# iclavera/learning_to_adapt

Hardware: AMD Instinct MI355X
Metric: controller-steps/sec (n_cand=2000, H=30, ens=5) (higher is better)
Workload: dtype f32

## Files before the change

learning_to_adapt_amd/csrc/l2a_mfma.h:

```cpp
#pragma once

#include <type_traits>

#include "l2a_kernels.h"

#ifndef L2A_XEARLY
#define L2A_XEARLY 1
#endif

#ifndef L2A_NW
#define L2A_NW 4
#endif

typedef unsigned int u32x4 __attribute__((ext_vector_type(4)));
__device__ __forceinline__ __amdgpu_buffer_rsrc_t l2a_rsrc(const void* base, long long bytes) {
    return __builtin_amdgcn_make_buffer_rsrc(const_cast<void*>(base), 0, (int)bytes, 0x00020000);
}
__device__ __forceinline__ f32x4 l2a_ldw(__amdgpu_buffer_rsrc_t rs, int voff, int soff) {
    return __builtin_bit_cast(f32x4, __builtin_amdgcn_raw_buffer_load_b128(rs, voff, soff, 0));
}

template <bool GACT>
__device__ __forceinline__ f32x4 l2a_actv(f32x4 v, int kind, float floor) {
    if (GACT) return l2a_act4(v, kind);
    v.x = l2a_max_nan(v.x, floor); v.y = l2a_max_nan(v.y, floor);
    v.z = l2a_max_nan(v.z, floor); v.w = l2a_max_nan(v.w, floor);
    return v;
}

__device__ __forceinline__ float l2a_sum_xor16(float x) {
    const unsigned int u = __float_as_uint(x);
    const auto r = __builtin_amdgcn_permlane16_swap(u, u, false, false);
    return __uint_as_float(r[0]) + __uint_as_float(r[1]);
}
__device__ __forceinline__ float l2a_sum_xor32(float x) {
    const unsigned int u = __float_as_uint(x);
    const auto r = __builtin_amdgcn_permlane32_swap(u, u, false, false);
    return __uint_as_float(r[0]) + __uint_as_float(r[1]);
}

#define L2A_MFMA4(a, b, c) __builtin_amdgcn_mfma_f32_4x4x1f32((a), (b), (c), 0, 0, 0)

#define L2A_OPAQUE(v) asm volatile("" : "+v"(v))

#ifndef L2A_TIMELINE
#define L2A_TS(slot)
#else
#define L2A_TS(slot)                                                                        \
    if (p.dbg && pairid == 0 && e < 8 && grp < 2) {                                         \
        unsigned long long ts_;                                                             \
        asm volatile("s_memtime %0\n\ts_waitcnt lgkmcnt(0)" : "=s"(ts_) : : "memory");       \
        if (lane == 0) p.dbg[(((long long)(grp * p.h + t) * 8 + e) * 8 + wave) * 16 + (slot)] = ts_; \
    }
#endif

#define L2A_STAGE_MFMA(CA, CB)                                                             \
    _Pragma("unroll") for (int ii = 0; ii < 4; ++ii)                                       \
        _Pragma("unroll") for (int nt = 0; nt < NT; ++nt)                                  \
            _Pragma("unroll") for (int tt = TW - 1; tt >= 0; --tt)    \
                acc[nt][tt] = L2A_MFMA(CA[tt][ii], CB[nt][ii], acc[nt][tt]);

#define L2A_STAGE(CA, CB, FA, FB, SOFF, IMM, GF)                                           \
    {                                                                                      \
        _Pragma("unroll") for (int tt = 0; tt < TW; ++tt)                                  \
            FA[tt] = l2a_ldw(rs, voff[tt] + (IMM), (SOFF));                                \
        _Pragma("unroll") for (int nt = 0; nt < NT; ++nt)                                  \
            FB[nt] = hin[(nt * HT + (GF)) * 64 + lane];                                    \
        L2A_STAGE_MFMA(CA, CB)                                                             \
         \
        __builtin_amdgcn_sched_group_barrier(0x100, NT, 0);                                \
        _Pragma("unroll") for (int tt = 0; tt < TW; ++tt) {                                \
            __builtin_amdgcn_sched_group_barrier(0x008, 4 * NT, 0);                        \
            __builtin_amdgcn_sched_group_barrier(0x020, 1, 0);                             \
        }                                                                                  \
        __builtin_amdgcn_sched_barrier(0);                                                 \
    }

#define L2A_PFT_MAX 6
#define L2A_PFT(TW_, OT_) ((OT_) <= 2 ? ((TW_) < L2A_PFT_MAX ? (TW_) : L2A_PFT_MAX) : ((TW_) < 2 ? (TW_) : 2))

template <int NT, int TW, int TPW, int OT, bool LAST>
__device__ __forceinline__ void l2a_hidden_gemm(__amdgpu_buffer_rsrc_t rs, __amdgpu_buffer_rsrc_t rsn,
                                                const int (&voff)[TPW], const int (&voffn)[TPW], int twn,
                                                int tile0, const f32x4* hin,
                                                f32x4 (&aA)[TPW], f32x4 (&aB)[TPW],
                                                f32x4 (&pfO)[TPW][OT], f32x4 (&acc)[NT][TPW], int lane,
                                                const float* bias_lds, f32x4 (&bias)[TPW], const int (&olane)[OT]) {
    constexpr int HT = L2A_NW * TPW;
    static_assert(HT % 4 == 0, "the k-group pipeline is unrolled by 4");
    f32x4 aC[TW], aD[TW], bA[NT], bB[NT], bC[NT], bD[NT];
#pragma unroll
    for (int nt = 0; nt < NT; ++nt) {
        bA[nt] = hin[(nt * HT + 0) * 64 + lane];
        bB[nt] = hin[(nt * HT + 1) * 64 + lane];
#pragma unroll
        for (int tt = 0; tt < TW; ++tt) acc[nt][tt] = (f32x4){0.f, 0.f, 0.f, 0.f};
    }
#pragma unroll
    for (int nt = 0; nt < NT; ++nt) { L2A_OPAQUE(bA[nt]); L2A_OPAQUE(bB[nt]); }
    __builtin_amdgcn_sched_barrier(0);

#pragma unroll 1
    for (int g = 0; g < HT - 4; g += 4) {
        const int soff = (g + 2) * 1024;
        L2A_STAGE(aA, bA, aC, bC, soff, 0, g + 2)
        L2A_STAGE(aB, bB, aD, bD, soff, 1024, g + 3)
        L2A_STAGE(aC, bC, aA, bA, soff, 2048, g + 4)
        L2A_STAGE(aD, bD, aB, bB, soff, 3072, g + 5)
    }
    L2A_STAGE(aA, bA, aC, bC, (HT - 2) * 1024, 0, HT - 2)
    L2A_STAGE(aB, bB, aD, bD, (HT - 2) * 1024, 1024, HT - 1)
    {
        if (LAST) {
#pragma unroll
            for (int tt = 0; tt < L2A_PFT(TW, OT); ++tt)
#pragma unroll
                for (int c = 0; c < OT; ++c)
                    if (((tt * OT + c) & 1) == 0)
                        pfO[tt][c] = l2a_ldw(rsn, olane[c] + (tile0 + tt) * 1024, c * HT * 1024);
        } else {
#pragma unroll
            for (int tt = 0; tt < TPW; ++tt)
                if (tt < twn) aA[tt] = l2a_ldw(rsn, voffn[tt], 0);
        }
        L2A_STAGE_MFMA(aC, bC)
        __builtin_amdgcn_sched_barrier(0);
    }
    {
#pragma unroll
        for (int tt = 0; tt < TW; ++tt) bias[tt] = *reinterpret_cast<const f32x4*>(bias_lds + 16 * tt);
        if (LAST) {
#pragma unroll
            for (int tt = 0; tt < L2A_PFT(TW, OT); ++tt)
#pragma unroll
                for (int c = 0; c < OT; ++c)
                    if (((tt * OT + c) & 1) == 1)
                        pfO[tt][c] = l2a_ldw(rsn, olane[c] + (tile0 + tt) * 1024, c * HT * 1024);
        } else {
#pragma unroll
            for (int tt = 0; tt < TPW; ++tt)
                if (tt < twn) aB[tt] = l2a_ldw(rsn, voffn[tt] + 1024, 0);
        }
        L2A_STAGE_MFMA(aD, bD)
        __builtin_amdgcn_sched_barrier(0);
    }
}

template <int NT, int TW, int TPW, int OT, int NPF, bool O4, class PF>
__device__ __forceinline__ void l2a_out_phase(const f32x4 (&hreg)[NT][TPW], f32x4 (&pfO)[TPW][OT],
                                              __amdgpu_buffer_rsrc_t rs_out, int tile0, PF prefetch,
                                              f32x4* pbuf, int chunk0, int lane, const int (&olane)[OT]) {
    constexpr int HT = L2A_NW * TPW;
    constexpr int CS = TPW / 2;
    constexpr int NCH = TW / CS;
    f32x4 a[TW][OT];
#pragma unroll
    for (int tt = 0; tt < TW; ++tt)
#pragma unroll
        for (int c = 0; c < OT; ++c)
            a[tt][c] = (tt < L2A_PFT(TW, OT)) ? pfO[tt][c]
                                              : l2a_ldw(rs_out, olane[c] + (tile0 + tt) * 1024, c * HT * 1024);
    prefetch();
    f32x4 acc[NCH][NT][OT];
#pragma unroll
    for (int ch = 0; ch < NCH; ++ch)
#pragma unroll
        for (int nt = 0; nt < NT; ++nt)
#pragma unroll
            for (int c = 0; c < OT; ++c) acc[ch][nt][c] = (f32x4){0.f, 0.f, 0.f, 0.f};
#pragma unroll
    for (int t2 = 0; t2 < CS; ++t2)
#pragma unroll
        for (int ii = 0; ii < 4; ++ii)
#pragma unroll
            for (int ch = 0; ch < NCH; ++ch)
#pragma unroll
                for (int nt = 0; nt < NT; ++nt)
#pragma unroll
                    for (int c = 0; c < OT; ++c)
                        acc[ch][nt][c] = (O4 && c == OT - 1)
                            ? L2A_MFMA4(a[ch * CS + t2][c][ii], hreg[nt][ch * CS + t2][ii], acc[ch][nt][c])
                            : L2A_MFMA(a[ch * CS + t2][c][ii], hreg[nt][ch * CS + t2][ii], acc[ch][nt][c]);
    {
        constexpr int NLATE = (TW - L2A_PFT(TW, OT)) * OT;
        constexpr int NMFMA = TW * 4 * NT * OT;
#pragma unroll
        for (int i = 0; i < NLATE; ++i) {
            __builtin_amdgcn_sched_group_barrier(0x020, 1, 0);
            __builtin_amdgcn_sched_group_barrier(0x008, 2, 0);
        }
        constexpr int PER = (NMFMA - 2 * NLATE) / NPF > 0 ? (NMFMA - 2 * NLATE) / NPF : 1;
#pragma unroll
        for (int i = 0; i < NPF; ++i) {
            __builtin_amdgcn_sched_group_barrier(0x008, PER, 0);
            __builtin_amdgcn_sched_group_barrier(0x020, 1, 0);
        }
    }
#pragma unroll
    for (int nt = 0; nt < NT; ++nt)
#pragma unroll
        for (int c = 0; c < OT; ++c)
            pbuf[((chunk0 * NT + nt) * OT + c) * 64 + lane] = (NCH == 2) ? acc[0][nt][c] + acc[NCH - 1][nt][c] : acc[0][nt][c];
}

template <int NT, int TPW, int OT, int KG0, bool GACT, int K0L = 4, bool N1 = false, bool O4 = false, bool FAN = false, bool WHOLE = false>
__global__ void __launch_bounds__(64 * L2A_NW) l2a_rollout_mfma_k(const L2AKParams p) {
    static_assert(!(FAN && WHOLE), "an instance is general, member fan or whole-tiles-only");
    constexpr bool NOHALF = FAN || WHOLE;
    constexpr int HT = L2A_NW * TPW;
    constexpr int TH = TPW / 2;
    static_assert(TPW % 2 == 0, "half members split a wave's tiles in two");
    constexpr int CST_BOUT = 32 * KG0 + 32 * OT;
    constexpr int CST_BHID = CST_BOUT + 16 * OT;
    constexpr int PS = L2A_NW * NT * OT * 64;
    const int NRM_SET = p.cst_set;
    const int LB = p.lb;
    extern __shared__ __attribute__((aligned(16))) char l2a_smem[];
    f32x4* buf0 = reinterpret_cast<f32x4*>(l2a_smem);
    f32x4* buf1 = buf0 + p.sa_elems;
    f32x4* pbase = buf0 + (LB > 1 ? LB : 2) * p.sa_elems;
    float* nrm = reinterpret_cast<float*>(buf0 + p.cst_off);

    const int tid = threadIdx.x;
    const int lane = tid & 63;
    const int wave = __builtin_amdgcn_readfirstlane(tid >> 6);
    const int jc = lane & 15;
    const int qq = lane >> 4;
    const int c0 = wave * TPW;
    int olane[OT];
#pragma unroll
    for (int c = 0; c < OT; ++c) olane[c] = ((O4 && c == OT - 1) ? ((lane & 48) | (lane & 3)) : lane) * 16;

    const int tail = p.split_from >= 0;
    const int in_tail = tail && (int)blockIdx.x >= p.split_from;
    const int split = FAN ? 3 : WHOLE ? 0 : (tail ? (in_tail ? p.split : 0) : p.split);
    const int n_tiles = p.m * p.tiles_per_env;
    const int n_pairs = tail ? n_tiles - p.split_from : n_tiles;
    int bid, grp, lpair, pairid;
    if (!tail && p.pl_units > 0) {
        const int hx = (int)blockIdx.x & 7, idx = (int)blockIdx.x >> 3;
        const int xcd = hx;
        const int f = p.pl_f, wide = p.pl_r * (f + 1);
        int u, k, xu;
        if (xcd < wide) { u = xcd / (f + 1); k = xcd - u * (f + 1); xu = f + 1; }
        else { const int y = xcd - wide; u = y / f; k = y - u * f; u += p.pl_r; xu = f; }
        const int su = (p.pl_w + xu - 1) / xu;
        const int j = k * su + idx;
        if (idx >= su || j >= p.pl_w) return;
        if (p.mode == L2A_MODE_PER_BLOCK) {
            grp = split ? j / p.tiles_per_env : 0;
            lpair = u * p.tiles_per_env + (j - grp * p.tiles_per_env);
        } else {
            grp = u;
            lpair = j;
        }
        bid = grp * n_pairs + lpair;
        pairid = lpair;
    } else if (!tail) {
        bid = l2a_logical_wg(blockIdx.x, gridDim.x);
        grp = split ? (bid / n_pairs) : 0;
        lpair = bid - grp * n_pairs;
        pairid = lpair;
    } else if (!in_tail) {
        bid = l2a_logical_wg(blockIdx.x, p.split_from);
        grp = 0; lpair = 0; pairid = bid;
    } else {
        bid = (int)blockIdx.x - p.split_from;
        grp = bid & 1; lpair = bid >> 1;
        pairid = p.split_from + lpair;
    }
#if defined(L2A_TIMELINE) || defined(L2A_WGREC)
    unsigned long long wg_t0_, wg_r0_;
    asm volatile("s_memtime %0\n\ts_memrealtime %1\n\ts_waitcnt lgkmcnt(0)" : "=s"(wg_t0_), "=s"(wg_r0_) : : "memory");
#endif
    const int env = pairid / p.tiles_per_env;
    const int tb = pairid - env * p.tiles_per_env;
    const int R = p.m * p.n;
    const int obs_dim = p.obs_dim, act_dim = p.act_dim;
    const int n_hidden = N1 ? 1 : p.n_hidden;

    int cand[NT], row[NT];
    bool valid[NT];
#pragma unroll
    for (int nt = 0; nt < NT; ++nt) {
        cand[nt] = p.c_lo + tb * (16 * NT) + nt * 16 + jc;
        valid[nt] = cand[nt] < p.c_hi;
        row[nt] = env * p.n + (valid[nt] ? cand[nt] : p.c_hi - 1);
    }

    const bool per_block = (p.mode == L2A_MODE_PER_BLOCK);
    const int e_loop = (p.mode == L2A_MODE_MEAN) ? p.n_sets : 1;
    const int e_half = (e_loop + 1) >> 1;
    const int e_shared = (!NOHALF && split == 2) ? e_half - 1 : -1;
    const int n_full = FAN ? 1 : (!split ? e_loop : (grp == 0 ? e_half - (split == 2 ? 1 : 0) : e_loop - e_half));
    const int n_seq = FAN ? 1 : n_full + (split == 2 ? 1 : 0);
    const int full0 = FAN ? grp : ((split && grp == 1) ? e_half : 0);
    auto seq = [&](int i) { return (i < n_full) ? full0 + i : e_shared; };
    auto set_base = [&](int e) { return p.wblk + (long long)(per_block ? env : e) * p.set_stride; };

    f32x4* xlds = reinterpret_cast<f32x4*>(nrm + p.n_cst * NRM_SET);
    for (int i = tid; i < n_seq * NRM_SET; i += 64 * L2A_NW) {
        const int s = i / NRM_SET;
        const int o = i - s * NRM_SET;
        const float* src = set_base(seq(s));
        float v;
        if (o < CST_BOUT) v = src[p.nm_off + o];
        else if (o < CST_BHID) v = src[p.pk_bout + (o - CST_BOUT)];
        else {
            const int l = (o - CST_BHID) / (16 * HT);
            v = src[p.raw_b[l] + (o - CST_BHID - l * 16 * HT)];
        }
        nrm[i] = v;
    }

    f32x4 st[NT][OT];
#pragma unroll
    for (int nt = 0; nt < NT; ++nt) {
        const float* orow = p.obs0 + (p.obs_per_row ? (long long)row[nt] : (long long)env) * obs_dim;
#pragma unroll
        for (int c = 0; c < OT; ++c)
#pragma unroll
            for (int ii = 0; ii < 4; ++ii) {
                const int dim = 16 * c + 4 * qq + ii;
                const float v = orow[dim < obs_dim ? dim : obs_dim - 1];
                st[nt][c][ii] = (dim < obs_dim) ? v : 0.0f;
            }
    }
    __syncthreads();

    const int ga0 = obs_dim >> 4;
    f32x4 av_next[NT][2];
    int aoff[NT][2][4];
#pragma unroll
    for (int nt = 0; nt < NT; ++nt)
#pragma unroll
        for (int s = 0; s < 2; ++s)
#pragma unroll
            for (int ii = 0; ii < 4; ++ii) {
                const int ka = 16 * (ga0 + s) + 4 * qq + ii - obs_dim;
                const bool in = (ka >= 0) && (ka < act_dim);
                aoff[nt][s][ii] = in ? (row[nt] * act_dim + ka) * 4 : 0x7ffffff0;
            }
    const long long a_step = (long long)R * act_dim;
    auto load_actions = [&](int t, f32x4 (&dst)[NT][2]) {
        const __amdgpu_buffer_rsrc_t ars = l2a_rsrc(p.actions + (long long)t * a_step, a_step * 4);
#pragma unroll
        for (int nt = 0; nt < NT; ++nt)
#pragma unroll
            for (int s = 0; s < 2; ++s)
#pragma unroll
                for (int ii = 0; ii < 4; ++ii)
                    dst[nt][s][ii] = __builtin_bit_cast(float, __builtin_amdgcn_raw_buffer_load_b32(ars, aoff[nt][s][ii], 0, 0));
    };
    f32x4 av[NT][2];
    float asq[NT];
    auto take_actions = [&](int t_fetch) {
#pragma unroll
        for (int nt = 0; nt < NT; ++nt) {
            av[nt][0] = av_next[nt][0];
            av[nt][1] = av_next[nt][1];
            float s = 0.0f;
#pragma unroll
            for (int ii = 0; ii < 4; ++ii) {
                s = fmaf(av[nt][0][ii], av[nt][0][ii], s);
                s = fmaf(av[nt][1][ii], av[nt][1][ii], s);
            }
            asq[nt] = s;
        }
        load_actions((t_fetch < p.h) ? t_fetch : p.h - 1, av_next);
    };
    load_actions(0, av_next);
    take_actions(1);

    float ret[NT];
#pragma unroll
    for (int nt = 0; nt < NT; ++nt) ret[nt] = p.ret_in ? p.ret_in[(long long)env * p.n + (valid[nt] ? cand[nt] : p.c_hi - 1)] : 0.0f;

    f32x4* hcur = buf0;
    f32x4* hoth = buf1;
    const float e_count = (float)e_loop;
    const float e_inv = 1.0f / e_count;
    double disc_pow = p.disc0;
    unsigned int spin_left = p.spin_limit;
    const unsigned int xtag0 = p.xtag;
    const __amdgpu_buffer_rsrc_t xrs = l2a_rsrc(p.xbuf, FAN ? (long long)n_pairs * e_loop * 2 * (NT * OT * 2 * 64 * 16)
                                                        : split ? (long long)n_pairs * 8 * (NT * OT * 2 * 64 * 16) : 16);

    constexpr int KG0P = (FAN && KG0 <= 2) ? KG0 : 1;
    f32x4 pfL0[KG0P][TPW];
    f32x4 pfA[TPW], pfB[TPW];
    f32x4 pfO[TPW][OT];
    int voff[TPW], voffh[TPW], voff0[TPW];
    const int tile0h = grp * (HT / 2) + wave * TH;
#pragma unroll
    for (int tt = 0; tt < TPW; ++tt) {
        voff[tt] = lane * 16 + (c0 + tt) * HT * 1024;
        voffh[tt] = lane * 16 + (tile0h + (tt < TH ? tt : 0)) * HT * 1024;
        voff0[tt] = lane * 16 + (c0 + tt) * KG0 * 1024;
    }
    const long long w0_bytes = (long long)HT * KG0 * 1024, wm_bytes = (long long)HT * HT * 1024,
                    wo_bytes = (long long)OT * HT * 1024;
    {
        const __amdgpu_buffer_rsrc_t r0 = l2a_rsrc(set_base(seq(0)) + p.pk_w0, w0_bytes);
#pragma unroll
        for (int g = 0; g < KG0P; ++g)
#pragma unroll
            for (int tt = 0; tt < TPW; ++tt) pfL0[g][tt] = l2a_ldw(r0, voff0[tt] + g * 1024, 0);
    }

    for (int t = 0; t < p.h; ++t) {
        f32x4 dsum[NT][OT], dgrp[NT][OT], qsh[NT][OT];
#pragma unroll
        for (int nt = 0; nt < NT; ++nt)
#pragma unroll
            for (int c = 0; c < OT; ++c) {
                dsum[nt][c] = (f32x4){0.f, 0.f, 0.f, 0.f};
                dgrp[nt][c] = (f32x4){0.f, 0.f, 0.f, 0.f};
                qsh[nt][c] = (f32x4){0.f, 0.f, 0.f, 0.f};
            }

        const unsigned int xtag = xtag0 + (unsigned int)(t + 1);
        constexpr int XREG = NT * OT * 2 * 64 * 16;
        auto xbase = [&](int g, int region) { return (((lpair * 2 + g) * 2 + (t & 1)) * 2 + region) * XREG + lane * 16; };
        auto xput = [&](int region, const f32x4 (&v)[NT][OT]) {
#pragma unroll
            for (int nt = 0; nt < NT; ++nt)
#pragma unroll
                for (int c = 0; c < OT; ++c)
#pragma unroll
                    for (int hh = 0; hh < 2; ++hh) {
                        u32x4 g;
                        g.x = xtag; g.y = __float_as_uint(v[nt][c][2 * hh]);
                        g.z = xtag; g.w = __float_as_uint(v[nt][c][2 * hh + 1]);
                        __builtin_amdgcn_raw_buffer_store_b128(g, xrs, xbase(grp, region) + ((nt * OT + c) * 2 + hh) * 1024, 0, L2A_SC1);
                    }
        };
        auto xget = [&](int region, f32x4 (&v)[NT][OT]) {
            bool ok = true;
#pragma unroll
            for (int nt = 0; nt < NT; ++nt)
#pragma unroll
                for (int c = 0; c < OT; ++c)
#pragma unroll
                    for (int hh = 0; hh < 2; ++hh) {
                        const u32x4 g = __builtin_amdgcn_raw_buffer_load_b128(
                            xrs, xbase(grp ^ 1, region) + ((nt * OT + c) * 2 + hh) * 1024, 0, L2A_SC1);
                        v[nt][c][2 * hh] = __uint_as_float(g.y);
                        v[nt][c][2 * hh + 1] = __uint_as_float(g.w);
                        ok = ok && (g.x == xtag) && (g.z == xtag);
                    }
            return ok;
        };

        bool xearly = false;
        u32x4 sw[2][NT][OT][2];
        for (int b0 = 0; b0 < n_seq; b0 += LB) {
            const int nb = (n_seq - b0 < LB) ? n_seq - b0 : LB;
            f32x4 hreg[NT][TPW];

            auto layer0 = [&](int j, auto last_tag) {
                constexpr bool last_l0 = decltype(last_tag)::value;
                const int i = b0 + j;
                const int e = seq(i);
                const float* wb = set_base(e);
                const float* nr = nrm + i * NRM_SET;
                const __amdgpu_buffer_rsrc_t rs_out = l2a_rsrc(wb + p.pk_wout, wo_bytes);
                L2A_TS(0)
                const __amdgpu_buffer_rsrc_t r0 = l2a_rsrc(wb + p.pk_w0, w0_bytes);
                f32x4 a[KG0][TPW];
#pragma unroll
                for (int g = 0; g < KG0; ++g)
#pragma unroll
                    for (int tt = 0; tt < TPW; ++tt)
                        a[g][tt] = (g < KG0P) ? pfL0[g < KG0P ? g : 0][tt] : l2a_ldw(r0, voff0[tt] + g * 1024, 0);
                L2A_TS(8)
                constexpr bool XPRE = (KG0 <= 2);
                auto norm_in = [&](int g, const f32x4& mu, const f32x4& iv, f32x4 (&x)[NT]) {
#pragma unroll
                    for (int nt = 0; nt < NT; ++nt) {
                        f32x4 sv = (f32x4){0.f, 0.f, 0.f, 0.f};
                        if (g < OT) sv = st[nt][g < OT ? g : 0];
                        f32x4 aa = (f32x4){0.f, 0.f, 0.f, 0.f};
                        if (g == ga0) aa = av[nt][0];
                        if (g == ga0 + 1) aa = av[nt][1];
#pragma unroll
                        for (int ii = 0; ii < 4; ++ii) x[nt][ii] = ((sv[ii] + aa[ii]) - mu[ii]) * iv[ii];
                    }
                };
                f32x4 xin[XPRE ? KG0 : 1][NT];
                if (XPRE) {
                    f32x4 mu[KG0], iv[KG0];
#pragma unroll
                    for (int g = 0; g < KG0; ++g) {
                        mu[g] = *reinterpret_cast<const f32x4*>(nr + 16 * g + 4 * qq);
                        iv[g] = *reinterpret_cast<const f32x4*>(nr + 16 * KG0 + 16 * g + 4 * qq);
                    }
                    __builtin_amdgcn_sched_barrier(0);
#pragma unroll
                    for (int g = 0; g < KG0; ++g) norm_in(g, mu[g], iv[g], xin[XPRE ? g : 0]);
                }
                f32x4 bias0[TPW];
#pragma unroll
                for (int tt = 0; tt < TPW; ++tt)
                    bias0[tt] = *reinterpret_cast<const f32x4*>(nr + CST_BHID + 16 * (c0 + tt) + 4 * qq);
                f32x4 acc[NT][TPW];
                auto l0_mfma = [&](auto npf_tag) {
                    constexpr int NPF = decltype(npf_tag)::value;
#pragma unroll
                    for (int nt = 0; nt < NT; ++nt)
#pragma unroll
                        for (int tt = 0; tt < TPW; ++tt) acc[nt][tt] = (f32x4){0.f, 0.f, 0.f, 0.f};
#pragma unroll
                    for (int g = 0; g < KG0; ++g) {
                        f32x4 xg[NT];
                        if (XPRE) {
#pragma unroll
                            for (int nt = 0; nt < NT; ++nt) xg[nt] = xin[XPRE ? g : 0][nt];
                        } else {
                            const f32x4 mu = *reinterpret_cast<const f32x4*>(nr + 16 * g + 4 * qq);
                            const f32x4 iv = *reinterpret_cast<const f32x4*>(nr + 16 * KG0 + 16 * g + 4 * qq);
                            norm_in(g, mu, iv, xg);
                        }
#pragma unroll
                        for (int ii = 0; ii < 4; ++ii) {
                            if (g == KG0 - 1 && ii >= K0L) continue;
#pragma unroll
                            for (int nt = 0; nt < NT; ++nt)
#pragma unroll
                                for (int tt = 0; tt < TPW; ++tt)
                                    acc[nt][tt] = L2A_MFMA(a[g][tt][ii], xg[nt][ii], acc[nt][tt]);
                        }
                    }
                    constexpr int NM = ((KG0 - 1) * 4 + K0L) * NT * TPW;
                    constexpr int PER = NM / (NPF > 0 ? NPF : 1) > 0 ? NM / (NPF > 0 ? NPF : 1) : 1;
                    __builtin_amdgcn_sched_group_barrier(0x020, (KG0 - KG0P) * TPW, 0);
#pragma unroll
                    for (int k = 0; k < NPF; ++k) {
                        __builtin_amdgcn_sched_group_barrier(0x008, PER, 0);
                        __builtin_amdgcn_sched_group_barrier(0x020, 1, 0);
                    }
                };
                if (N1) {
#pragma unroll
                    for (int tt = 0; tt < L2A_PFT(TPW, OT); ++tt)
#pragma unroll
                        for (int c = 0; c < OT; ++c)
                            pfO[tt][c] = l2a_ldw(rs_out, olane[c] + (c0 + tt) * 1024, c * HT * 1024);
                    l0_mfma(std::integral_constant<int, L2A_PFT(TPW, OT) * OT>{});
                } else if (!last_l0) {
                    const __amdgpu_buffer_rsrc_t r0n = l2a_rsrc(set_base(seq(i + 1)) + p.pk_w0, w0_bytes);
#pragma unroll
                    for (int g = 0; g < KG0P; ++g)
#pragma unroll
                        for (int tt = 0; tt < TPW; ++tt) pfL0[g][tt] = l2a_ldw(r0n, voff0[tt] + g * 1024, 0);
                    l0_mfma(std::integral_constant<int, KG0P * TPW>{});
                } else {
                    const int e0 = seq(b0);
                    const __amdgpu_buffer_rsrc_t rs1 = l2a_rsrc(set_base(e0) + p.pk_wmid, wm_bytes);
                    const bool next_half = !NOHALF && (e0 == e_shared) && n_hidden == 2;
                    if (next_half) {
#pragma unroll
                        for (int tt = 0; tt < TH; ++tt) {
                            pfA[tt] = l2a_ldw(rs1, voffh[tt], 0);
                            pfB[tt] = l2a_ldw(rs1, voffh[tt] + 1024, 0);
                        }
                        l0_mfma(std::integral_constant<int, 2 * TH>{});
                    } else {
#pragma unroll
                        for (int tt = 0; tt < TPW; ++tt) {
                            pfA[tt] = l2a_ldw(rs1, voff[tt], 0);
                            pfB[tt] = l2a_ldw(rs1, voff[tt] + 1024, 0);
                        }
                        l0_mfma(std::integral_constant<int, 2 * TPW>{});
                    }
                }
                L2A_TS(9)
#pragma unroll
                for (int tt = 0; tt < TPW; ++tt) {
#pragma unroll
                    for (int nt = 0; nt < NT; ++nt)
                        hreg[nt][tt] = l2a_actv<GACT>(acc[nt][tt] + bias0[tt], p.hidden_act, p.hid_floor);
                }
                L2A_TS(10)
                if (!N1) {
                    f32x4* hdst = (LB > 1) ? buf0 + j * p.sa_elems : hcur;
#pragma unroll
                    for (int tt = 0; tt < TPW; ++tt)
#pragma unroll
                        for (int nt = 0; nt < NT; ++nt) hdst[(nt * HT + c0 + tt) * 64 + lane] = hreg[nt][tt];
                }
                L2A_TS(1)
            };

            auto member = [&](int j, auto last_tag) {
                constexpr bool last_set = decltype(last_tag)::value;
                const int i = b0 + j;
                const int e = seq(i);
                const bool is_half = !NOHALF && last_set && (e == e_shared);
                const float* wb = set_base(e);
                const float* nr = nrm + i * NRM_SET;
                const __amdgpu_buffer_rsrc_t rs_out = l2a_rsrc(wb + p.pk_wout, wo_bytes);
                f32x4* pb = (LB > 1) ? pbase + j * PS : hoth;
                L2A_TS(2)
                if (!N1) {
                    f32x4 acc[NT][TPW], bias[TPW];
                    for (int l = 1; last_set && l < n_hidden - 1; ++l) {
                        const float* wl = wb + p.pk_wmid + (long long)(l - 1) * p.pk_wmid_stride;
                        const bool next_half = is_half && (l == n_hidden - 2);
                        l2a_hidden_gemm<NT, TPW, TPW, OT, false>(l2a_rsrc(wl, wm_bytes), l2a_rsrc(wl + p.pk_wmid_stride, wm_bytes),
                                                                 voff, next_half ? voffh : voff, next_half ? TH : TPW, 0,
                                                                 hcur, pfA, pfB, pfO, acc, lane,
                                                                 nr + CST_BHID + l * (16 * HT) + 16 * c0 + 4 * qq, bias, olane);
#pragma unroll
                        for (int tt = 0; tt < TPW; ++tt) {
#pragma unroll
                            for (int nt = 0; nt < NT; ++nt)
                                hoth[(nt * HT + c0 + tt) * 64 + lane] = l2a_actv<GACT>(acc[nt][tt] + bias[tt], p.hidden_act, p.hid_floor);
                        }
                        __syncthreads();
                        f32x4* tmp = hcur; hcur = hoth; hoth = tmp;
                    }
                    if (LB == 1) pb = hoth;
                    L2A_TS(15)
                    const f32x4* hin = (LB > 1) ? buf0 + j * p.sa_elems : hcur;
                    const __amdgpu_buffer_rsrc_t rs_last =
                        l2a_rsrc(wb + p.pk_wmid + (long long)(n_hidden - 2) * p.pk_wmid_stride, wm_bytes);
                    const float* bl = nr + CST_BHID + (n_hidden - 1) * (16 * HT);
                    if (!is_half) {
                        l2a_hidden_gemm<NT, TPW, TPW, OT, true>(rs_last, rs_out, voff, voff, TPW, c0, hin, pfA, pfB, pfO,
                                                                acc, lane, bl + 16 * c0 + 4 * qq, bias, olane);
#pragma unroll
                        for (int tt = 0; tt < TPW; ++tt) {
#pragma unroll
                            for (int nt = 0; nt < NT; ++nt)
                                hreg[nt][tt] = l2a_actv<GACT>(acc[nt][tt] + bias[tt], p.hidden_act, p.hid_floor);
                        }
                    } else {
                        l2a_hidden_gemm<NT, TH, TPW, OT, true>(rs_last, rs_out, voffh, voffh, TH, tile0h, hin, pfA, pfB,
                                                               pfO, acc, lane, bl + 16 * tile0h + 4 * qq, bias, olane);
#pragma unroll
                        for (int tt = 0; tt < TH; ++tt) {
#pragma unroll
                            for (int nt = 0; nt < NT; ++nt)
                                hreg[nt][tt] = l2a_actv<GACT>(acc[nt][tt] + bias[tt], p.hidden_act, p.hid_floor);
                        }
                    }
                }
                L2A_TS(3)
                if (last_set) {
                    const __amdgpu_buffer_rsrc_t r0n = l2a_rsrc(set_base(seq((i + 1 < n_seq) ? i + 1 : 0)) + p.pk_w0, w0_bytes);
                    auto pf_l0 = [&]() {
#pragma unroll
                        for (int g = 0; g < KG0P; ++g)
#pragma unroll
                            for (int tt = 0; tt < TPW; ++tt) pfL0[g][tt] = l2a_ldw(r0n, voff0[tt] + g * 1024, 0);
                    };
                    if (is_half) l2a_out_phase<NT, TH, TPW, OT, KG0P * TPW, O4>(hreg, pfO, rs_out, tile0h, pf_l0, pb, wave, lane, olane);
                    else l2a_out_phase<NT, TPW, TPW, OT, KG0P * TPW, O4>(hreg, pfO, rs_out, c0, pf_l0, pb, wave, lane, olane);
                } else {
                    const int en = seq(i + 1);
                    const __amdgpu_buffer_rsrc_t rsn = l2a_rsrc(set_base(en) + p.pk_wmid, wm_bytes);
                    if (!NOHALF && en == e_shared) {
                        l2a_out_phase<NT, TPW, TPW, OT, 2 * TH, O4>(hreg, pfO, rs_out, c0, [&]() {
#pragma unroll
                            for (int tt = 0; tt < TH; ++tt) {
                                pfA[tt] = l2a_ldw(rsn, voffh[tt], 0);
                                pfB[tt] = l2a_ldw(rsn, voffh[tt] + 1024, 0);
                            }
                        }, pb, wave, lane, olane);
                    } else {
                        l2a_out_phase<NT, TPW, TPW, OT, 2 * TPW, O4>(hreg, pfO, rs_out, c0, [&]() {
#pragma unroll
                            for (int tt = 0; tt < TPW; ++tt) {
                                pfA[tt] = l2a_ldw(rsn, voff[tt], 0);
                                pfB[tt] = l2a_ldw(rsn, voff[tt] + 1024, 0);
                            }
                        }, pb, wave, lane, olane);
                    }
                }
                L2A_TS(4)
            };
            for (int j = 0; j + 1 < nb; ++j) layer0(j, std::false_type{});
            layer0(nb - 1, std::true_type{});
            if (!N1) __syncthreads();
            for (int j = 0; j + 1 < nb; ++j) member(j, std::false_type{});
            member(nb - 1, std::true_type{});

            __syncthreads();
            constexpr bool XE_OK = L2A_XEARLY && !NOHALF && NT == 1 && OT <= 2 && KG0 <= 2;
            const bool xe = XE_OK && split == 2 && nb >= 2 && b0 + nb == n_seq;
            for (int jj = 0; jj < nb; ++jj) {
                const int j = (xe && wave == 0) ? (jj == 0 ? nb - 1 : jj - 1) : jj;
                const int i = b0 + j;
                const int e = seq(i);
                const bool is_half = !NOHALF && (e == e_shared);
                const float* nr = nrm + i * NRM_SET;
                const f32x4* pb = (LB > 1) ? pbase + j * PS : hoth;
                L2A_TS(5)
                if (e == e_half && !split) {
#pragma unroll
                    for (int nt = 0; nt < NT; ++nt)
#pragma unroll
                        for (int c = 0; c < OT; ++c) {
                            dsum[nt][c] = dgrp[nt][c];
                            dgrp[nt][c] = (f32x4){0.f, 0.f, 0.f, 0.f};
                        }
                }
#pragma unroll
                for (int c = 0; c < OT; ++c) {
                    f32x4 part[L2A_NW][NT];
#pragma unroll
                    for (int ch = 0; ch < L2A_NW; ++ch)
#pragma unroll
                        for (int nt = 0; nt < NT; ++nt) part[ch][nt] = pb[((ch * NT + nt) * OT + c) * 64 + lane];
                    const f32x4 bias = *reinterpret_cast<const f32x4*>(nr + CST_BOUT + 16 * c + 4 * qq);
                    const f32x4 omu = *reinterpret_cast<const f32x4*>(nr + 32 * KG0 + 16 * c + 4 * qq);
                    const f32x4 osd = *reinterpret_cast<const f32x4*>(nr + 32 * KG0 + 16 * OT + 16 * c + 4 * qq);
                    __builtin_amdgcn_sched_barrier(0);
#pragma unroll
                    for (int nt = 0; nt < NT; ++nt) {
                        static_assert(L2A_NW == 4, "the canonical tree below is written out for four waves");
                        f32x4 s = (part[0][nt] + part[1][nt]) + (part[2][nt] + part[3][nt]);
                        if (is_half) {
                            qsh[nt][c] = s;
                        } else {
                            if (O4 && c == OT - 1) {
#pragma unroll
                                for (int ii = 0; ii < 4; ++ii) s[ii] = l2a_sum_xor32(l2a_sum_xor16(s[ii]));
                            }
                            s = l2a_actv<GACT>(s + bias, p.output_act, p.out_floor);
                            if (FAN) dgrp[nt][c] = s * osd + omu;
                            else dgrp[nt][c] += s * osd + omu;
                        }
                    }
                }
                if (!NOHALF && split == 2 && i == n_full - 1 && wave == (XE_OK ? 1 : 0)) xput(0, dgrp);
                if (xe && wave == 0 && jj == 0) xput(1, qsh);
                if (xe && wave == 3 && jj == nb - 1) {
#pragma unroll
                    for (int r = 0; r < 2; ++r)
#pragma unroll
                        for (int nt = 0; nt < NT; ++nt)
#pragma unroll
                            for (int c = 0; c < OT; ++c)
#pragma unroll
                                for (int hh = 0; hh < 2; ++hh)
                                    sw[r][nt][c][hh] = (r == 1 || e_loop > 1)
                                        ? __builtin_amdgcn_raw_buffer_load_b128(xrs, xbase(grp ^ 1, r) + ((nt * OT + c) * 2 + hh) * 1024, 0, L2A_SC1)
                                        : (u32x4){xtag, 0u, xtag, 0u};
                }
                L2A_TS(6)
            }
            if (xe) xearly = true;
            if (N1) { f32x4* tmp = hcur; hcur = hoth; hoth = tmp; }
        }

        { const int e = 7; L2A_TS(9) }
        float asq_t[NT];
#pragma unroll
        for (int nt = 0; nt < NT; ++nt) asq_t[nt] = asq[nt];
        if (FAN) {
            constexpr int XREGF = NT * OT * 2 * 64 * 16;
            auto fbase = [&](int g) { return ((lpair * e_loop + g) * 2 + (t & 1)) * XREGF + lane * 16; };
            if (wave == 0) {
#pragma unroll
                for (int nt = 0; nt < NT; ++nt)
#pragma unroll
                    for (int c = 0; c < OT; ++c) {
#pragma unroll
                        for (int hh = 0; hh < 2; ++hh) {
                            u32x4 g;
                            g.x = xtag; g.y = __float_as_uint(dgrp[nt][c][2 * hh]);
                            g.z = xtag; g.w = __float_as_uint(dgrp[nt][c][2 * hh + 1]);
                            __builtin_amdgcn_raw_buffer_store_b128(g, xrs, fbase(grp) + ((nt * OT + c) * 2 + hh) * 1024, 0, L2A_SC1);
                        }
                        xlds[((grp * NT + nt) * OT + c) * 64 + lane] = dgrp[nt][c];
                    }
            }
            { const int e = 7; L2A_TS(11) }
            take_actions(t + 2);
            for (int k = wave; k < e_loop - 1; k += L2A_NW) {
                int g2 = grp + 1 + k;
                if (g2 >= e_loop) g2 -= e_loop;
                f32x4 oth[NT][OT];
                while (true) {
                    bool ok = true;
#pragma unroll
                    for (int nt = 0; nt < NT; ++nt)
#pragma unroll
                        for (int c = 0; c < OT; ++c)
#pragma unroll
                            for (int hh = 0; hh < 2; ++hh) {
                                const u32x4 g = __builtin_amdgcn_raw_buffer_load_b128(
                                    xrs, fbase(g2) + ((nt * OT + c) * 2 + hh) * 1024, 0, L2A_SC1);
                                oth[nt][c][2 * hh] = __uint_as_float(g.y);
                                oth[nt][c][2 * hh + 1] = __uint_as_float(g.w);
                                ok = ok && (g.x == xtag) && (g.z == xtag);
                            }
                    if (__all(ok)) break;
                    if (spin_left == 0) {
                        if (lane == 0) __hip_atomic_fetch_or(p.status, 1u, __ATOMIC_RELAXED, __HIP_MEMORY_SCOPE_SYSTEM);
                        break;
                    }
                    --spin_left;
                    __builtin_amdgcn_s_sleep(4);
                }
#pragma unroll
                for (int nt = 0; nt < NT; ++nt)
#pragma unroll
                    for (int c = 0; c < OT; ++c) xlds[((g2 * NT + nt) * OT + c) * 64 + lane] = oth[nt][c];
            }
            { const int e = 7; L2A_TS(12) }
            __syncthreads();
            { const int e = 7; L2A_TS(13) }
#pragma unroll
            for (int nt = 0; nt < NT; ++nt)
#pragma unroll
                for (int c = 0; c < OT; ++c) {
                    dsum[nt][c] = (f32x4){0.f, 0.f, 0.f, 0.f};
                    dgrp[nt][c] = (f32x4){0.f, 0.f, 0.f, 0.f};
                }
            {
                constexpr int EMAX = 8;
                f32x4 v[EMAX][NT][OT];
#pragma unroll
                for (int e = 0; e < EMAX; ++e) {
                    const int es = e < e_loop ? e : e_loop - 1;
#pragma unroll
                    for (int nt = 0; nt < NT; ++nt)
#pragma unroll
                        for (int c = 0; c < OT; ++c) v[e][nt][c] = xlds[((es * NT + nt) * OT + c) * 64 + lane];
                }
                __builtin_amdgcn_sched_barrier(0);
#pragma unroll
                for (int e = 0; e < EMAX; ++e)
#pragma unroll
                    for (int nt = 0; nt < NT; ++nt)
#pragma unroll
                        for (int c = 0; c < OT; ++c) {
                            if (e < e_half) dsum[nt][c] += v[e][nt][c];
                            else if (e < e_loop) dgrp[nt][c] += v[e][nt][c];
                        }
            }
        } else if (!WHOLE && split) {
            if (wave == 0 && !xearly) {
                if (split == 2) xput(1, qsh);
                else xput(0, dgrp);
            }
            { const int e = 7; L2A_TS(11) }
            take_actions(t + 2);
            if (xearly && wave == 3) {
                while (true) {
                    bool ok = true;
#pragma unroll
                    for (int r = 0; r < 2; ++r)
#pragma unroll
                        for (int nt = 0; nt < NT; ++nt)
#pragma unroll
                            for (int c = 0; c < OT; ++c)
#pragma unroll
                                for (int hh = 0; hh < 2; ++hh)
                                    ok = ok && (sw[r][nt][c][hh].x == xtag) && (sw[r][nt][c][hh].z == xtag);
                    if (__all(ok)) break;
                    if (spin_left == 0) {
                        if (lane == 0) __hip_atomic_fetch_or(p.status, 1u, __ATOMIC_RELAXED, __HIP_MEMORY_SCOPE_SYSTEM);
                        break;
                    }
                    --spin_left;
                    __builtin_amdgcn_s_sleep(4);
#pragma unroll
                    for (int r = 0; r < 2; ++r)
#pragma unroll
                        for (int nt = 0; nt < NT; ++nt)
#pragma unroll
                            for (int c = 0; c < OT; ++c)
#pragma unroll
                                for (int hh = 0; hh < 2; ++hh)
                                    if (r == 1 || e_loop > 1)
                                        sw[r][nt][c][hh] = __builtin_amdgcn_raw_buffer_load_b128(
                                            xrs, xbase(grp ^ 1, r) + ((nt * OT + c) * 2 + hh) * 1024, 0, L2A_SC1);
                }
#pragma unroll
                for (int r = 0; r < 2; ++r)
#pragma unroll
                    for (int nt = 0; nt < NT; ++nt)
#pragma unroll
                        for (int c = 0; c < OT; ++c) {
                            f32x4 v;
                            v[0] = __uint_as_float(sw[r][nt][c][0].y); v[1] = __uint_as_float(sw[r][nt][c][0].w);
                            v[2] = __uint_as_float(sw[r][nt][c][1].y); v[3] = __uint_as_float(sw[r][nt][c][1].w);
                            xlds[((r * NT + nt) * OT + c) * 64 + lane] = v;
                        }
                { const int e = 7; L2A_TS(12) }
            }
            if (wave == 0 && !xearly) {
                f32x4 oth[2][NT][OT];
#pragma unroll
                for (int nt = 0; nt < NT; ++nt)
#pragma unroll
                    for (int c = 0; c < OT; ++c) {
                        oth[0][nt][c] = (f32x4){0.f, 0.f, 0.f, 0.f};
                        oth[1][nt][c] = (f32x4){0.f, 0.f, 0.f, 0.f};
                    }
                const bool want0 = (split == 1) || (e_loop > 1);
                unsigned int spins = 0;
                auto give_up = [&]() {
                    ++spins;
                    if (spin_left == 0) {
                        if (lane == 0) __hip_atomic_fetch_or(p.status, 1u, __ATOMIC_RELAXED, __HIP_MEMORY_SCOPE_SYSTEM);
                        return true;
                    }
                    --spin_left;
                    return false;
                };
                while (true) {
                    bool ok = true;
                    if (split == 2) ok = xget(1, oth[1]);
                    if (want0) ok = xget(0, oth[0]) && ok;
                    if (__all(ok) || give_up()) break;
                    __builtin_amdgcn_s_sleep(4);
                }
#pragma unroll
                for (int k = 0; k < 2; ++k)
#pragma unroll
                    for (int nt = 0; nt < NT; ++nt)
#pragma unroll
                        for (int c = 0; c < OT; ++c) xlds[((k * NT + nt) * OT + c) * 64 + lane] = oth[k][nt][c];
                { const int e = 7; L2A_TS(12) }
#ifdef L2A_TIMELINE
                if (p.dbg && pairid == 0 && lane == 0) p.dbg[(((long long)(grp * p.h + t) * 8 + 7) * 8 + wave) * 16 + 14] = spins;
#endif
            }
            { const int e = 7; L2A_TS(10) }
            __syncthreads();
            { const int e = 7; L2A_TS(13) }
            const float* nrs = nrm + (n_seq - 1) * NRM_SET;
            {
                f32x4 cb[OT], cm[OT], cs[OT], og[NT][OT], oq[NT][OT];
#pragma unroll
                for (int c = 0; c < OT; ++c) {
                    cb[c] = *reinterpret_cast<const f32x4*>(nrs + CST_BOUT + 16 * c + 4 * qq);
                    cm[c] = *reinterpret_cast<const f32x4*>(nrs + 32 * KG0 + 16 * c + 4 * qq);
                    cs[c] = *reinterpret_cast<const f32x4*>(nrs + 32 * KG0 + 16 * OT + 16 * c + 4 * qq);
#pragma unroll
                    for (int nt = 0; nt < NT; ++nt) {
                        og[nt][c] = xlds[((0 * NT + nt) * OT + c) * 64 + lane];
                        oq[nt][c] = xlds[((1 * NT + nt) * OT + c) * 64 + lane];
                    }
                }
                __builtin_amdgcn_sched_barrier(0);
#pragma unroll
                for (int c = 0; c < OT; ++c)
#pragma unroll
                    for (int nt = 0; nt < NT; ++nt) {
                        f32x4 ga = (grp == 0) ? dgrp[nt][c] : og[nt][c];
                        const f32x4 gb = (grp == 0) ? og[nt][c] : dgrp[nt][c];
                        if (split == 2) {
                            f32x4 s = qsh[nt][c] + oq[nt][c];
                            if (O4 && c == OT - 1) {
#pragma unroll
                                for (int ii = 0; ii < 4; ++ii) s[ii] = l2a_sum_xor32(l2a_sum_xor16(s[ii]));
                            }
                            s = l2a_actv<GACT>(s + cb[c], p.output_act, p.out_floor);
                            ga += s * cs[c] + cm[c];
                        }
                        dsum[nt][c] = ga;
                        dgrp[nt][c] = gb;
                    }
            }
        } else {
            take_actions(t + 2);
        }
#pragma unroll
        for (int nt = 0; nt < NT; ++nt)
#pragma unroll
            for (int c = 0; c < OT; ++c) dsum[nt][c] += dgrp[nt][c];

        const float disc_t = (float)disc_pow;
        disc_pow *= p.discount;
#pragma unroll
        for (int nt = 0; nt < NT; ++nt) {
            float plin = ((qq == 0) ? p.rw.alive : 0.0f) - (p.rw.ctrl_coef != 0.0f ? p.rw.ctrl_coef * asq_t[nt] : 0.0f);
            float psq = 0.0f;
#pragma unroll
            for (int c = 0; c < OT; ++c) {
                f32x4 d = dsum[nt][c];
                if (e_loop > 1) {
#pragma unroll
                    for (int ii = 0; ii < 4; ++ii) {
                        const float q = d[ii] * e_inv;
                        const float qc = fmaf(fmaf(-q, e_count, d[ii]), e_inv, q);
                        d[ii] = (fabsf(q) < INFINITY) ? qc : q;
                    }
                }
                f32x4 nx = st[nt][c] + d;
                if (c == OT - 1) {
#pragma unroll
                    for (int ii = 0; ii < 4; ++ii)
                        if (16 * c + 4 * qq + ii >= obs_dim) nx[ii] = 0.0f;
                }
#pragma unroll
                for (int ii = 0; ii < 4; ++ii) {
                    const int dim = 16 * c + 4 * qq + ii;
                    if (p.rw.w_vel != 0.0f && dim == p.rw.vel_index)
                        plin += p.rw.w_vel * (d[ii] + (st[nt][c][ii] - st[nt][c][ii])) * p.rw.inv_dt;
                    const bool in_dist = (p.rw.dist_coef != 0.0f) && (dim >= p.rw.dist_index) &&
                                         (dim < p.rw.dist_index + 3) && (dim < obs_dim);
                    psq += in_dist ? nx[ii] * nx[ii] : 0.0f;
                }
                st[nt][c] = nx;
            }
            plin = l2a_sum_xor32(l2a_sum_xor16(plin));
            psq = l2a_sum_xor32(l2a_sum_xor16(psq));
            float r = plin;
            if (p.rw.dist_coef != 0.0f) r -= p.rw.dist_coef * sqrtf(psq);
            ret[nt] = fmaf(disc_t, r, ret[nt]);
        }
        { const int e = 7; L2A_TS(7) }
    }

    if (wave == 0 && grp == 0) {
        unsigned long long key = 0ull;
#pragma unroll
        for (int nt = 0; nt < NT; ++nt) {
            if (valid[nt] && qq == 0) {
                if (p.returns_out) p.returns_out[(long long)env * p.n + cand[nt]] = ret[nt];
                const unsigned long long k = l2a_key_pack(ret[nt], p.cand_offset + cand[nt]);
                key = (k > key) ? k : key;
            }
            if (p.state_out && valid[nt]) {
                float* srow = p.state_out + ((long long)env * p.n + cand[nt]) * obs_dim;
#pragma unroll
                for (int c = 0; c < OT; ++c)
#pragma unroll
                    for (int ii = 0; ii < 4; ++ii) {
                        const int dim = 16 * c + 4 * qq + ii;
                        if (dim < obs_dim) srow[dim] = st[nt][c][ii];
                    }
            }
        }
        if (p.best_key) {
#pragma unroll
            for (int off = 32; off >= 1; off >>= 1) {
                const unsigned int hi = __shfl_xor((unsigned int)(key >> 32), off);
                const unsigned int lo = __shfl_xor((unsigned int)(key & 0xffffffffu), off);
                const unsigned long long other = ((unsigned long long)hi << 32) | lo;
                key = (other > key) ? other : key;
            }
            if (lane == 0) {
                if (key != 0ull) atomicMax(p.best_key + env, key);
                l2a_publish_result(p, p.done_total > 0 ? p.done_total : n_tiles);
            }
        }
    }
#if defined(L2A_TIMELINE) || defined(L2A_WGREC)
    if (p.dbg && wave == 0 && lane == 0 && grp < 2) {
        unsigned long long wg_t1_, wg_r1_;
        unsigned int xcc_;
        asm volatile("s_memtime %0\n\ts_memrealtime %1\n\ts_waitcnt lgkmcnt(0)" : "=s"(wg_t1_), "=s"(wg_r1_) : : "memory");
        asm volatile("s_getreg_b32 %0, hwreg(HW_REG_XCC_ID)" : "=s"(xcc_));
        unsigned long long* r = p.dbg + (long long)2 * p.h * 8 * 8 * 16 + (long long)(grp * n_tiles + pairid) * 6;
        r[0] = wg_t0_; r[1] = wg_t1_; r[2] = xcc_; r[3] = blockIdx.x; r[4] = wg_r0_; r[5] = wg_r1_;
    }
#endif
}
```

Before: 704.0.

## Deepen weight prefetch ring for half-width member's last hidden layer

For the half-width (shared) member's last hidden layer, the unused half of the A/B prefetch registers now serves as a four-k-group-ahead ring of eight buffers instead of two, using a k-loop unrolled by eight. The prefetch offsets for that member are reorganised so the initial loads fill all four ring slots with k-groups 0-3. This hides more global weight-load latency behind MFMA work, at the cost of extra register pressure and more loads issued up front.

```diff
diff --git a/learning_to_adapt_amd/csrc/l2a_mfma.h b/learning_to_adapt_amd/csrc/l2a_mfma.h
--- a/learning_to_adapt_amd/csrc/l2a_mfma.h
+++ b/learning_to_adapt_amd/csrc/l2a_mfma.h
@@ -6,6 +6,10 @@
 
 #ifndef L2A_XEARLY
 #define L2A_XEARLY 1
+#endif
+
+#ifndef L2A_HALFRING
+#define L2A_HALFRING 1
 #endif
 
 #ifndef L2A_NW
@@ -100,6 +104,62 @@
     for (int nt = 0; nt < NT; ++nt) { L2A_OPAQUE(bA[nt]); L2A_OPAQUE(bB[nt]); }
     __builtin_amdgcn_sched_barrier(0);
 
+    if constexpr (L2A_HALFRING && TW < TPW) {
+        static_assert(LAST && 2 * TW == TPW && HT % 8 == 0, "the deep ring is the half member's last hidden layer");
+        f32x4 r0[TW], r1[TW], r2[TW], r3[TW], r4[TW], r5[TW], r6[TW], r7[TW];
+#pragma unroll
+        for (int tt = 0; tt < TW; ++tt) { r0[tt] = aA[tt]; r1[tt] = aA[TW + tt]; r2[tt] = aB[tt]; r3[tt] = aB[TW + tt]; }
+#pragma unroll 1
+        for (int g = 0; g < HT - 8; g += 8) {
+            const int soff = (g + 4) * 1024, soff2 = (g + 8) * 1024;
+            L2A_STAGE(r0, bA, r4, bC, soff, 0, g + 2)
+            L2A_STAGE(r1, bB, r5, bD, soff, 1024, g + 3)
+            L2A_STAGE(r2, bC, r6, bA, soff, 2048, g + 4)
+            L2A_STAGE(r3, bD, r7, bB, soff, 3072, g + 5)
+            L2A_STAGE(r4, bA, r0, bC, soff2, 0, g + 6)
+            L2A_STAGE(r5, bB, r1, bD, soff2, 1024, g + 7)
+            L2A_STAGE(r6, bC, r2, bA, soff2, 2048, g + 8)
+            L2A_STAGE(r7, bD, r3, bB, soff2, 3072, g + 9)
+        }
+        L2A_STAGE(r0, bA, r4, bC, (HT - 4) * 1024, 0, HT - 6)
+        L2A_STAGE(r1, bB, r5, bD, (HT - 4) * 1024, 1024, HT - 5)
+        L2A_STAGE(r2, bC, r6, bA, (HT - 4) * 1024, 2048, HT - 4)
+        L2A_STAGE(r3, bD, r7, bB, (HT - 4) * 1024, 3072, HT - 3)
+#define L2A_STAGE_B(CA, CB, FB, GF)                                                        \
+        {                                                                                  \
+            _Pragma("unroll") for (int nt = 0; nt < NT; ++nt)                              \
+                FB[nt] = hin[(nt * HT + (GF)) * 64 + lane];                                \
+            L2A_STAGE_MFMA(CA, CB)                                                         \
+            __builtin_amdgcn_sched_barrier(0);                                             \
+        }
+        L2A_STAGE_B(r4, bA, bC, HT - 2)
+        L2A_STAGE_B(r5, bB, bD, HT - 1)
+#undef L2A_STAGE_B
+        {
+#pragma unroll
+            for (int tt = 0; tt < L2A_PFT(TW, OT); ++tt)
+#pragma unroll
+                for (int c = 0; c < OT; ++c)
+                    if (((tt * OT + c) & 1) == 0)
+                        pfO[tt][c] = l2a_ldw(rsn, olane[c] + (tile0 + tt) * 1024, c * HT * 1024);
+            L2A_STAGE_MFMA(r6, bC)
+            __builtin_amdgcn_sched_barrier(0);
+        }
+        {
+#pragma unroll
+            for (int tt = 0; tt < TW; ++tt) bias[tt] = *reinterpret_cast<const f32x4*>(bias_lds + 16 * tt);
+#pragma unroll
+            for (int tt = 0; tt < L2A_PFT(TW, OT); ++tt)
+#pragma unroll
+                for (int c = 0; c < OT; ++c)
+                    if (((tt * OT + c) & 1) == 1)
+                        pfO[tt][c] = l2a_ldw(rsn, olane[c] + (tile0 + tt) * 1024, c * HT * 1024);
+            L2A_STAGE_MFMA(r7, bD)
+            __builtin_amdgcn_sched_barrier(0);
+        }
+        return;
+    }
+
 #pragma unroll 1
     for (int g = 0; g < HT - 4; g += 4) {
         const int soff = (g + 2) * 1024;
@@ -121,7 +181,7 @@
         } else {
 #pragma unroll
             for (int tt = 0; tt < TPW; ++tt)
-                if (tt < twn) aA[tt] = l2a_ldw(rsn, voffn[tt], 0);
+                if (L2A_HALFRING || tt < twn) aA[tt] = l2a_ldw(rsn, voffn[tt], 0);
         }
         L2A_STAGE_MFMA(aC, bC)
         __builtin_amdgcn_sched_barrier(0);
@@ -139,7 +199,7 @@
         } else {
 #pragma unroll
             for (int tt = 0; tt < TPW; ++tt)
-                if (tt < twn) aB[tt] = l2a_ldw(rsn, voffn[tt] + 1024, 0);
+                if (L2A_HALFRING || tt < twn) aB[tt] = l2a_ldw(rsn, voffn[tt] + ((L2A_HALFRING && twn < TPW) ? 2048 : 1024), 0);
         }
         L2A_STAGE_MFMA(aD, bD)
         __builtin_amdgcn_sched_barrier(0);
@@ -395,7 +455,8 @@
 #pragma unroll
     for (int tt = 0; tt < TPW; ++tt) {
         voff[tt] = lane * 16 + (c0 + tt) * HT * 1024;
-        voffh[tt] = lane * 16 + (tile0h + (tt < TH ? tt : 0)) * HT * 1024;
+        voffh[tt] = L2A_HALFRING ? lane * 16 + (tile0h + (tt < TH ? tt : tt - TH)) * HT * 1024 + (tt < TH ? 0 : 1024)
+                                 : lane * 16 + (tile0h + (tt < TH ? tt : 0)) * HT * 1024;
         voff0[tt] = lane * 16 + (c0 + tt) * KG0 * 1024;
     }
     const long long w0_bytes = (long long)HT * KG0 * 1024, wm_bytes = (long long)HT * HT * 1024,
@@ -559,12 +620,13 @@
                     const __amdgpu_buffer_rsrc_t rs1 = l2a_rsrc(set_base(e0) + p.pk_wmid, wm_bytes);
                     const bool next_half = !NOHALF && (e0 == e_shared) && n_hidden == 2;
                     if (next_half) {
-#pragma unroll
-                        for (int tt = 0; tt < TH; ++tt) {
+                        constexpr int TWP = L2A_HALFRING ? TPW : TH;
+#pragma unroll
+                        for (int tt = 0; tt < TWP; ++tt) {
                             pfA[tt] = l2a_ldw(rs1, voffh[tt], 0);
-                            pfB[tt] = l2a_ldw(rs1, voffh[tt] + 1024, 0);
-                        }
-                        l0_mfma(std::integral_constant<int, 2 * TH>{});
+                            pfB[tt] = l2a_ldw(rs1, voffh[tt] + (L2A_HALFRING ? 2048 : 1024), 0);
+                        }
+                        l0_mfma(std::integral_constant<int, 2 * TWP>{});
                     } else {
 #pragma unroll
                         for (int tt = 0; tt < TPW; ++tt) {
@@ -661,11 +723,12 @@
                     const int en = seq(i + 1);
                     const __amdgpu_buffer_rsrc_t rsn = l2a_rsrc(set_base(en) + p.pk_wmid, wm_bytes);
                     if (!NOHALF && en == e_shared) {
-                        l2a_out_phase<NT, TPW, TPW, OT, 2 * TH, O4>(hreg, pfO, rs_out, c0, [&]() {
-#pragma unroll
-                            for (int tt = 0; tt < TH; ++tt) {
+                        constexpr int TWP = L2A_HALFRING ? TPW : TH;
+                        l2a_out_phase<NT, TPW, TPW, OT, 2 * TWP, O4>(hreg, pfO, rs_out, c0, [&]() {
+#pragma unroll
+                            for (int tt = 0; tt < TWP; ++tt) {
                                 pfA[tt] = l2a_ldw(rsn, voffh[tt], 0);
-                                pfB[tt] = l2a_ldw(rsn, voffh[tt] + 1024, 0);
+                                pfB[tt] = l2a_ldw(rsn, voffh[tt] + (L2A_HALFRING ? 2048 : 1024), 0);
                             }
                         }, pb, wave, lane, olane);
                     } else {
```

Measured after the change: 704.0 (median of 4 runs). About the same (-0.0%).
